# TritonDataCenter/containerpilot

Hardware: NVIDIA H100
Metric: events/sec through Bus.Publish (deliveries/s = 32-byte records landed in subscriber mailboxes) (higher is better)
Workload: dtype u8

## Files before the change

containerpilot_b200/csrc/cpbus.cu:

```cuda
#include "cpbus_kernels.cuh"

#include <algorithm>
#include <chrono>
#include <cstdio>
#include <cstdlib>
#include <cstring>
#include <deque>
#include <mutex>
#include <new>
#include <string>
#include <thread>
#include <unordered_map>
#include <vector>

using namespace cpbus_dev;

namespace {

thread_local char g_cuda_err[256] = "";

#define CK(call)                                                                                   \
  do {                                                                                             \
    cudaError_t e_ = (call);                                                                       \
    if (e_ != cudaSuccess) {                                                                       \
// ... 43 lines not shown
  uint32_t N = 0, R = 0, B = 0, K = 0;
  int store = CPBUS_STORE_V8;
  bool lossless = false, use_digest = false;

  cpbus_event* d_ring = nullptr;
  SubCtl* d_ctl = nullptr;
  DevTimer* d_timers = nullptr;
  DevStats* d_stats = nullptr;
  uint64_t* d_pow = nullptr;
  unsigned char* d_desc = nullptr;
  unsigned long long* d_desc_ready = nullptr;
  unsigned long long launch_seq = 0;
  cpbus_event* d_batch_local = nullptr;
  cpbus_event* d_admit_batch = nullptr;
  static constexpr int kPrefetch = 3;
  cpbus_event* d_prefetch[kPrefetch] = {};
  const void* pf_ptr[kPrefetch] = {};
  size_t pf_n[kPrefetch] = {};
  unsigned long long pf_seq[kPrefetch] = {};
  int pf_next = 0;
  std::vector<void*> shared_owned, shared_mapped;
  unsigned long long* d_pf_state = nullptr;
  cpbus_event* d_pf_buf = nullptr;
  unsigned int* h_err = nullptr;
  unsigned int* d_err = nullptr;
  uint32_t stream_spin_us = 0;
  DevPubAcct* d_acct = nullptr;
  DevPubAcct* h_acct = nullptr;
  std::deque<DbgItem> dbg_pending;
  PairCounter pub_pairs;
  cpbus_event* d_drain = nullptr; size_t drain_cap = 0;
  uint2* d_drain_idx = nullptr; size_t drain_idx_cap = 0;
  unsigned long long* d_ready_lb = nullptr; size_t ready_lb_tiles = 0;
  cpbus_ready* d_ready = nullptr; uint32_t* d_ready_slot = nullptr; size_t ready_stage_cap = 0;
  unsigned long long* h_ready_hdr = nullptr;
  unsigned long long* d_ready_hdr = nullptr;
  uint32_t subs_per_warp = 0;
  uint32_t order_block = 0;
  bool order_heavy_first = true;
  bool pdl = true;
  int h2d_spin_us = 30;
  bool zero_copy = false;
  cudaEvent_t launched = nullptr;
  int hints = -1;
  static constexpr int kFoldSlots = 8;
  unsigned long long* d_fold = nullptr;
  cudaEvent_t fold_done[kFoldSlots] = {};
  uint32_t fold_next = 0;
  static constexpr int kStage = 8;
  static constexpr int kEpoch = 4;
  static constexpr int kDevSlots = 64, kDevEpoch = 16;
  cpbus_event* d_stage = nullptr;
  cudaEvent_t epoch_done[kDevSlots / kDevEpoch] = {};
  uint32_t dev_slot = 0;
  cpbus_event* h_batch[kStage] = {};
  cudaEvent_t h2d_done[kStage] = {};
  cudaEvent_t consumed[kStage] = {};
  cudaStream_t copy_stream = nullptr;
  cudaStream_t result_stream = nullptr;
  DevResultSlot* d_result = nullptr;
  DevResultSlot* h_result = nullptr;
  cudaEvent_t result_done[8] = {};
  uint32_t result_next = 0;
  DevStats* h_stats = nullptr;
  unsigned long long* h_fold = nullptr;
  int cur = 0;
  size_t n_staged = 0;

  std::vector<uint32_t> h_mask;
  std::vector<uint8_t> h_active;
  std::vector<uint8_t> h_npairs;
  uint2* d_pairs = nullptr;
  uint32_t n_paired = 0;
  uint32_t* d_order = nullptr;
  uint32_t n_order = 0, n_filtered = 0;
  bool order_dirty = true;
  int use_order = 1;
  std::vector<size_t> oneshot_idx;
  std::vector<HostTimer> h_timers;
  uint32_t n_next = 0, n_active = 0, n_timers = 0;
  uint64_t min_period = UINT64_MAX;

  uint64_t now = 0, last_watermark = 0, seq = 0;
  uint64_t room_lb = 0;

  int dbg_head = -1, dbg_tail = 0;
  cpbus_event dbg[10]{};

  std::unordered_map<std::string, uint32_t> intern;
  std::vector<std::string> sources;
  size_t intern_bytes = 0;
  struct EphSlot { std::string s; uint32_t gen = 0; bool live = false; };
  std::vector<EphSlot> eph;
  std::unordered_map<std::string, uint32_t> eph_map;
  uint32_t eph_next = 0;
  uint64_t eph_live = 0, eph_recycled = 0;
  std::vector<cpbus_stream*> streams;

  cpbus_stats_t st{};
  std::mutex mu;
};

namespace {
// ... 459 lines not shown
  ALLOC(b->d_pf_buf, (size_t)kStreamPrefetch * B * sizeof(cpbus_event)); ALLOC(b->d_pf_state, 64);
  ALLOC(b->d_acct, sizeof(DevPubAcct));
  if (cudaMemsetAsync(b->d_pf_state, 0, 64, b->stream) != cudaSuccess ||
      cudaMemsetAsync(b->d_acct, 0, sizeof(DevPubAcct), b->stream) != cudaSuccess) return fail(CPBUS_ECUDA);
  if (cudaHostAlloc((void**)&b->h_err, 64, cudaHostAllocMapped) != cudaSuccess) return fail(CPBUS_ENOMEM);
  memset(b->h_err, 0, 64);
  if (cudaHostGetDevicePointer((void**)&b->d_err, b->h_err, 0) != cudaSuccess) return fail(CPBUS_ECUDA);
  if (cudaMallocHost((void**)&b->h_acct, offsetof(DevPubAcct, pair_key)) != cudaSuccess) return fail(CPBUS_ENOMEM);
  for (int i = 0; i < cpbus::kPrefetch; i++) ALLOC(b->d_prefetch[i], (size_t)B * sizeof(cpbus_event));
  ALLOC(b->d_result, sizeof(DevResultSlot) * kResultRing * kResultSub);
  if (cudaMemsetAsync(b->d_result, 0, sizeof(DevResultSlot) * kResultRing * kResultSub, b->stream) != cudaSuccess) return fail(CPBUS_ECUDA);
  if (cudaMallocHost((void**)&b->h_result, sizeof(DevResultSlot) * 8 * kResultSub) != cudaSuccess) return fail(CPBUS_ENOMEM);
  for (int i = 0; i < 8; i++)
    if (cudaEventCreateWithFlags(&b->result_done[i], cudaEventDisableTiming) != cudaSuccess) return fail(CPBUS_ECUDA);
#undef ALLOC
  if (cudaMallocHost((void**)&b->h_stats, sizeof(DevStats)) != cudaSuccess) return fail(CPBUS_ENOMEM);
  if (cudaMallocHost((void**)&b->h_fold, 32 * cpbus::kFoldSlots) != cudaSuccess) return fail(CPBUS_ENOMEM);
  for (int i = 0; i < cpbus::kFoldSlots; i++)
    if (cudaEventCreateWithFlags(&b->fold_done[i], cudaEventDisableTiming) != cudaSuccess) return fail(CPBUS_ECUDA);
  bool ok = cudaMemsetAsync(b->d_ctl, 0, N * sizeof(SubCtl), b->stream) == cudaSuccess &&
            cudaMemsetAsync(b->d_stats, 0, sizeof(DevStats), b->stream) == cudaSuccess &&
            (!K || cudaMemsetAsync(b->d_timers, 0xFF, N * K * sizeof(DevTimer), b->stream) == cudaSuccess) &&
            cudaStreamSynchronize(b->stream) == cudaSuccess;
  if (!ok) return fail(CPBUS_ECUDA);
  {
    std::vector<uint64_t> pw(kPowTableLen);
    uint64_t x = 1;
    for (uint32_t i = 0; i < kPowTableLen; i++) { pw[i] = x; x *= kDigestP; }
    if (cudaMemcpyAsync(b->d_pow, pw.data(), kPowTableLen * 8, cudaMemcpyHostToDevice, b->stream) != cudaSuccess ||
        cudaStreamSynchronize(b->stream) != cudaSuccess) return fail(CPBUS_ECUDA);
  }
  b->h_mask.assign(N, 0);
  b->h_active.assign(N, 0);
  b->intern.emplace(std::string(), 0u);
  b->sources.emplace_back();
  *out = b;
  return CPBUS_OK;
} CPBUS_CATCH

int cpbus_destroy(cpbus_t* b) try {
  if (!b) return CPBUS_EINVAL;
  cudaSetDevice(b->device);
  if (b->stream) cudaStreamSynchronize(b->stream);
  while (!b->streams.empty()) cpbus_stream_close(b->streams.back());
  cudaFree(b->d_ring); cudaFree(b->d_ctl); cudaFree(b->d_order); cudaFree(b->d_pairs);
  cudaFree(b->d_timers); cudaFree(b->d_stats); cudaFree(b->d_fold); cudaFree(b->d_pow); cudaFree(b->d_desc); cudaFree(b->d_desc_ready);
  if (b->copy_stream) cudaStreamSynchronize(b->copy_stream);
  if (b->result_stream) { cudaStreamSynchronize(b->result_stream); cudaStreamDestroy(b->result_stream); }
  for (int i = 0; i < cpbus::kStage; i++) {
    if (b->h_batch[i]) cudaFreeHost(b->h_batch[i]);
    if (b->h2d_done[i]) cudaEventDestroy(b->h2d_done[i]);
    if (b->consumed[i]) cudaEventDestroy(b->consumed[i]);
  }
  cudaFree(b->d_stage);
  for (int i = 0; i < cpbus::kDevSlots / cpbus::kDevEpoch; i++) if (b->epoch_done[i]) cudaEventDestroy(b->epoch_done[i]);
  if (b->copy_stream) cudaStreamDestroy(b->copy_stream);
  if (b->launched) cudaEventDestroy(b->launched);
  cudaFree(b->d_drain); cudaFree(b->d_drain_idx);
  cudaFree(b->d_ready_lb); cudaFree(b->d_ready); cudaFree(b->d_ready_slot);
  if (b->h_ready_hdr) cudaFreeHost(b->h_ready_hdr);
  cudaFree(b->d_result); cudaFree(b->d_batch_local); cudaFree(b->d_admit_batch); cudaFree(b->d_pf_buf); cudaFree(b->d_pf_state); cudaFree(b->d_acct);
  if (b->h_err) cudaFreeHost(b->h_err);
  if (b->h_acct) cudaFreeHost(b->h_acct);
  for (int i = 0; i < cpbus::kPrefetch; i++) cudaFree(b->d_prefetch[i]);
  for (void* p : b->shared_mapped) cudaIpcCloseMemHandle(p);
  for (void* p : b->shared_owned) cudaFree(p);
// ... 42 lines not shown
  b->eph_map.emplace(std::move(key), slot);
  *source_id = CPBUS_EPHEMERAL_BIT | ((e.gen & 0x7FFFu) << 16) | slot;
  return CPBUS_OK;
} CPBUS_CATCH

int cpbus_source(cpbus_t* b, uint32_t id, char* out, size_t cap, size_t* len) try {
  if (!b) return CPBUS_EINVAL;
  if (id & CPBUS_EPHEMERAL_BIT) {
    const uint32_t slot = id & 0xFFFFu, gen = (id >> 16) & 0x7FFFu;
    if (slot >= b->eph.size() || !b->eph[slot].live || (b->eph[slot].gen & 0x7FFFu) != gen) return CPBUS_ENOENT;
    const std::string& s = b->eph[slot].s;
    if (len) *len = s.size();
    if (out && cap) memcpy(out, s.data(), std::min(cap, s.size()));
    return CPBUS_OK;
  }
  if (id >= b->sources.size()) return CPBUS_ENOENT;
  const std::string& s = b->sources[id];
  if (len) *len = s.size();
  if (out && cap) memcpy(out, s.data(), std::min(cap, s.size()));
  return CPBUS_OK;
} CPBUS_CATCH

int cpbus_subscribe_many(cpbus_t* b, const uint32_t* masks, uint32_t n, uint32_t* first_sub_id) try {
  if (!b || !n) return CPBUS_EINVAL;
  if ((uint64_t)b->n_next + n > b->N) return CPBUS_ENOSPC;
  int rc = dev_guard(b); if (rc) return rc;
  if ((rc = flush_staged(b, b->now))) return rc;
  const uint32_t first = b->n_next;
  std::vector<SubCtl> blocks(n);
  memset(blocks.data(), 0, (size_t)n * sizeof(SubCtl));
  for (uint32_t i = 0; i < n; i++) {
    b->h_mask[first + i] = (masks ? masks[i] : CPBUS_MASK_ALL) & CPBUS_MASK_ALL;
    blocks[i].mask = b->h_mask[first + i] | kActiveBit;
    b->h_active[first + i] = 1;
    if (b->h_mask[first + i] != CPBUS_MASK_ALL) b->n_filtered++;
  }
  CK(cudaMemcpyAsync(b->d_ctl + first, blocks.data(), (size_t)n * sizeof(SubCtl), cudaMemcpyHostToDevice, b->stream));
  CK(cudaStreamSynchronize(b->stream));
  b->n_next += n; b->n_active += n; b->order_dirty = true;
  if (first_sub_id) *first_sub_id = b->cfg.sub_id_base + first;
  return CPBUS_OK;
} CPBUS_CATCH

int cpbus_subscribe(cpbus_t* b, uint32_t mask, uint32_t* sub_id) { return cpbus_subscribe_many(b, &mask, 1, sub_id); }

static int push_mask_words(cpbus* b, uint32_t first, uint32_t n);

int cpbus_subscribe_pairs(cpbus_t* b, uint32_t mask, const cpbus_pair* pairs, uint32_t n_pairs, uint32_t* sub_id) try {
  if (!b || n_pairs > CPBUS_MAX_PAIRS || (n_pairs && !pairs)) return CPBUS_EINVAL;
  for (uint32_t j = 0; j < n_pairs; j++) if (pairs[j].code >= CPBUS_N_CODES) return CPBUS_EINVAL;
  uint2 row[CPBUS_MAX_PAIRS];
  uint32_t used = 0;
  for (uint32_t j = 0; j < n_pairs; j++)
    if (!((mask >> pairs[j].code) & 1u)) row[used++] = make_uint2(pairs[j].code, pairs[j].source_id);
  if (used == 0) return cpbus_subscribe_many(b, &mask, 1, sub_id);
  int rc = dev_guard(b); if (rc) return rc;
  if (!b->d_pairs) {
    if (cudaMalloc((void**)&b->d_pairs, (size_t)b->N * CPBUS_MAX_PAIRS * sizeof(uint2)) != cudaSuccess) {
      snprintf(g_cuda_err, sizeof(g_cuda_err), "cudaMalloc(pair tables) failed");
      return CPBUS_ENOMEM;
    }
    CK(cudaMemsetAsync(b->d_pairs, 0xFF, (size_t)b->N * CPBUS_MAX_PAIRS * sizeof(uint2), b->stream));
    b->h_npairs.assign(b->N, 0);
  }
  uint32_t id = 0;
  if ((rc = cpbus_subscribe_many(b, &mask, 1, &id))) return rc;
  const uint32_t l = id - b->cfg.sub_id_base;
  for (uint32_t j = used; j < CPBUS_MAX_PAIRS; j++) row[j] = make_uint2(kPairNone, kPairNone);
  CK(cudaMemcpyAsync(b->d_pairs + (size_t)l * CPBUS_MAX_PAIRS, row, sizeof(row), cudaMemcpyHostToDevice, b->stream));
// ... 696 lines not shown
  if (*(volatile unsigned int*)b->h_err) return CPBUS_ETIMEDOUT;
  if (!st->h_agree) {
    StreamAgreeResult *h = nullptr, *d = nullptr;
    CK(cudaHostAlloc((void**)&h, sizeof(StreamAgreeResult), cudaHostAllocMapped));
    if (cudaHostGetDevicePointer((void**)&d, h, 0) != cudaSuccess) { cudaFreeHost(h); CK(cudaGetLastError()); return CPBUS_ECUDA; }
    st->h_agree = h; st->d_agree = d;
  }
  if (!st->agree_done) CK(cudaEventCreateWithFlags(&st->agree_done, cudaEventDisableTiming));
  const unsigned long long r = st->agree_round + 1;
  stream_agree_kernel<<<1, kStreamMaxConsumers, 0, b->stream>>>(st->ack, st->n_consumers, r, b->stream_spin_us, st->d_agree, b->d_err);
  CK(cudaGetLastError());
  b->st.kernel_launches++;
  st->agree_round = r; st->offered = false;
  CK(cudaEventRecord(st->agree_done, b->stream));
  CK(cudaEventSynchronize(st->agree_done));
  const volatile StreamAgreeResult* res = st->h_agree;
  if (res->status) return CPBUS_ETIMEDOUT;
  if (res->stalled) return CPBUS_EAGAIN;
  *m = res->m;
  return CPBUS_OK;
} CPBUS_CATCH

static int read_cursors(cpbus* b, uint32_t l, uint64_t* tail, uint64_t* head, uint64_t* lost = nullptr) {
  SubCtl c{};
  CK(cudaMemcpyAsync(&c, b->d_ctl + l, sizeof(SubCtl), cudaMemcpyDeviceToHost, b->stream));
  CK(cudaStreamSynchronize(b->stream));
  *tail = c.tail;
  *head = (!b->lossless && c.tail > b->R && c.tail - b->R > c.head) ? c.tail - b->R : c.head;
  if (lost) *lost = *head - c.head;
  return CPBUS_OK;
}

static int copy_slots(cpbus* b, uint32_t l, uint64_t from, size_t n, cpbus_event* out) {
  const cpbus_event* ring = b->d_ring + (size_t)l * b->R;
  const uint32_t s0 = (uint32_t)(from & (b->R - 1));
  const size_t first = std::min<size_t>(n, b->R - s0);
  if (first) CK(cudaMemcpyAsync(out, ring + s0, first * sizeof(cpbus_event), cudaMemcpyDeviceToHost, b->stream));
  if (n > first) CK(cudaMemcpyAsync(out + first, ring, (n - first) * sizeof(cpbus_event), cudaMemcpyDeviceToHost, b->stream));
  CK(cudaStreamSynchronize(b->stream));
  return CPBUS_OK;
}

int cpbus_drain(cpbus_t* b, uint32_t sub_id, cpbus_event* out, size_t cap, size_t* n, uint64_t* lost) try {
  if (!b || !n || (!out && cap)) return CPBUS_EINVAL;
  const uint32_t l = sub_id - b->cfg.sub_id_base;
  if (sub_id < b->cfg.sub_id_base || l >= b->n_next) return CPBUS_ENOENT;
  std::lock_guard<std::mutex> g(b->mu);
  int rc = dev_guard(b); if (rc) return rc;
  uint64_t tail = 0, head = 0;
  uint64_t gone = 0;
  if ((rc = read_cursors(b, l, &tail, &head, &gone))) return rc;
  if (lost) *lost = gone;
  const size_t take = (size_t)std::min<uint64_t>(tail - head, cap);
  if (take && (rc = copy_slots(b, l, head, take, out))) return rc;
  head += take;
  CK(cudaMemcpyAsync(&b->d_ctl[l].head, &head, 8, cudaMemcpyHostToDevice, b->stream));
  CK(cudaStreamSynchronize(b->stream));
  *n = take;
  return CPBUS_OK;
} CPBUS_CATCH

int cpbus_drain_many(cpbus_t* b, uint32_t first_sub, uint32_t n, cpbus_event* out, size_t cap, uint32_t* offsets,
                     uint32_t* counts, size_t* total) try {
  if (!b || !n || !out || !cap || !offsets || !counts || !total || cap > 0xFFFFFFFFull) return CPBUS_EINVAL;
  const uint32_t l = first_sub - b->cfg.sub_id_base;
  if (first_sub < b->cfg.sub_id_base || (uint64_t)l + n > b->n_next) return CPBUS_ENOENT;
  std::lock_guard<std::mutex> g(b->mu);
// ... 11 lines not shown
  b->st.kernel_launches++;
  std::vector<uint2> idx(n);
  CK(cudaMemcpyAsync(idx.data(), b->d_drain_idx, (size_t)n * sizeof(uint2), cudaMemcpyDeviceToHost, b->stream));
  CK(cudaStreamSynchronize(b->stream));
  size_t tot = 0, hi = 0;
  for (uint32_t i = 0; i < n; i++) {
    offsets[i] = idx[i].x; counts[i] = idx[i].y; tot += idx[i].y;
    hi = std::max<size_t>(hi, (size_t)idx[i].x + idx[i].y);
  }
  if (hi) CK(cudaMemcpyAsync(out, b->d_drain, hi * sizeof(cpbus_event), cudaMemcpyDeviceToHost, b->stream));
  CK(cudaStreamSynchronize(b->stream));
  *total = tot;
  return CPBUS_OK;
} CPBUS_CATCH

int cpbus_drain_ready(cpbus_t* b, uint32_t first_sub, uint32_t n, uint32_t start_sub, cpbus_event* out, size_t cap,
                      cpbus_ready* ready, size_t ready_cap, size_t* n_ready, size_t* total, uint32_t* next_sub) try {
  if (!b || !out || !ready || !n_ready || !total || !next_sub || !n || !ready_cap) return CPBUS_EINVAL;
  if (cap < b->R || cap > 0xFFFFFFFFull) return CPBUS_EINVAL;
  if (start_sub < first_sub || start_sub - first_sub >= n) return CPBUS_EINVAL;
  const uint32_t l = first_sub - b->cfg.sub_id_base;
  if (first_sub < b->cfg.sub_id_base || (uint64_t)l + n > b->n_next) return CPBUS_ENOENT;
  std::lock_guard<std::mutex> g(b->mu);
  int rc = dev_guard(b); if (rc) return rc;
  const size_t rcap = std::min<size_t>(ready_cap, n);
  const uint32_t tiles = (n + kReadyTile - 1) / kReadyTile;
  if (b->drain_cap < cap) {
    cudaFree(b->d_drain); b->d_drain = nullptr; b->drain_cap = 0;
    CK(cudaMalloc((void**)&b->d_drain, cap * sizeof(cpbus_event))); b->drain_cap = cap;
  }
  if (b->ready_stage_cap < rcap) {
    cudaFree(b->d_ready); cudaFree(b->d_ready_slot); b->d_ready = nullptr; b->d_ready_slot = nullptr; b->ready_stage_cap = 0;
    CK(cudaMalloc((void**)&b->d_ready, rcap * sizeof(cpbus_ready)));
    CK(cudaMalloc((void**)&b->d_ready_slot, rcap * sizeof(uint32_t)));
    b->ready_stage_cap = rcap;
  }
  if (b->ready_lb_tiles < tiles) {
    cudaFree(b->d_ready_lb); b->d_ready_lb = nullptr; b->ready_lb_tiles = 0;
    CK(cudaMalloc((void**)&b->d_ready_lb, (kReadyLbOffset + (size_t)tiles) * sizeof(unsigned long long)));
    b->ready_lb_tiles = tiles;
  }
  if (!b->h_ready_hdr) {
    unsigned long long *h = nullptr, *d = nullptr;
    CK(cudaHostAlloc((void**)&h, 64, cudaHostAllocMapped));
    if (cudaHostGetDevicePointer((void**)&d, h, 0) != cudaSuccess) { cudaFreeHost(h); CK(cudaGetLastError()); return CPBUS_ECUDA; }
    b->h_ready_hdr = h; b->d_ready_hdr = d;
  }
  CK(cudaMemsetAsync(b->d_ready_lb + kReadyHdrWords, 0, (kReadyLbOffset - kReadyHdrWords + (size_t)tiles) * sizeof(unsigned long long),
                     b->stream));
  const uint32_t rot = start_sub - first_sub;
  drain_ready_scan_kernel<<<tiles, kThreads, 0, b->stream>>>(b->d_ctl, l, n, rot, b->R, b->lossless ? 1u : 0u, b->cfg.sub_id_base,
                                                              cap, rcap, b->d_ready_lb, b->d_ready, b->d_ready_slot);
  CK(cudaGetLastError());
  const uint32_t gather_grid = (uint32_t)std::min<size_t>((size_t)b->sm_count * 4, (rcap + kWarpsPerCta - 1) / kWarpsPerCta);
  drain_ready_gather_kernel<<<gather_grid, kThreads, 0, b->stream>>>(b->d_ring, b->R, b->cfg.sub_id_base, b->d_ready,
                                                                      b->d_ready_slot, b->d_ready_lb, b->d_drain, b->d_ready_hdr);
  CK(cudaGetLastError());
  b->st.kernel_launches += 2;
  CK(cudaStreamSynchronize(b->stream));
  const size_t nr = (size_t)b->h_ready_hdr[0], tot = (size_t)b->h_ready_hdr[1];
  const uint64_t cut = b->h_ready_hdr[2];
  if (nr) {
    CK(cudaMemcpyAsync(ready, b->d_ready, nr * sizeof(cpbus_ready), cudaMemcpyDeviceToHost, b->stream));
    CK(cudaMemcpyAsync(out, b->d_drain, tot * sizeof(cpbus_event), cudaMemcpyDeviceToHost, b->stream));
    CK(cudaStreamSynchronize(b->stream));
  }
  *n_ready = nr; *total = tot;
  *next_sub = cut >= n ? start_sub : first_sub + (uint32_t)((rot + cut) % n);
  return CPBUS_OK;
} CPBUS_CATCH

int cpbus_consume_all(cpbus_t* b) try {
  if (!b) return CPBUS_EINVAL;
  std::lock_guard<std::mutex> g(b->mu);
  int rc = dev_guard(b); if (rc) return rc;
  if (b->n_next) {
    const uint32_t threads = 256, grid = std::min<uint32_t>((b->n_next + threads - 1) / threads, (uint32_t)b->sm_count * 8);
    consume_all_kernel<<<grid, threads, 0, b->stream>>>(b->d_ctl, b->n_next);
    CK(cudaGetLastError());
    b->st.kernel_launches++;
  }
  b->room_lb = b->R;
  return CPBUS_OK;
} CPBUS_CATCH

int cpbus_peek_window(cpbus_t* b, uint32_t sub_id, cpbus_event* out, size_t cap, size_t* n) try {
  if (!b || !n || (!out && cap)) return CPBUS_EINVAL;
  const uint32_t l = sub_id - b->cfg.sub_id_base;
// ... 173 lines not shown
```

containerpilot_b200/csrc/cpbus_kernels.cuh:

```cuda
#pragma once
#include <cstdint>
#include <cuda_runtime.h>

#include "../../include/cpbus.h"

namespace cpbus_dev {

constexpr int kWarpsPerCta = 8;
constexpr int kThreads = kWarpsPerCta * 32;
#ifndef CPBUS_CTAS_PER_SM
#define CPBUS_CTAS_PER_SM 4
#endif
#ifndef CPBUS_SWIZZLE
#define CPBUS_SWIZZLE 2
#endif
#ifndef CPBUS_TICKS_REG
#define CPBUS_TICKS_REG 1
#endif
#ifndef CPBUS_COLD_EARLY
#define CPBUS_COLD_EARLY 1
#endif
#ifndef CPBUS_UNROLL2
#define CPBUS_UNROLL2 1
#endif
// ... 29 lines not shown
};
constexpr uint64_t kTimerIdle = ~0ull;

constexpr int kStatSlots = 256;
struct __align__(32) DevStatSlot { unsigned long long deliveries, ticks, pad[2]; };
struct DevStats {
  DevStatSlot slot[kStatSlots];
  unsigned long long admit_overflow, overwritten;
  unsigned long long admit_max_used;
  unsigned long long admit_deficit;
};

constexpr uint32_t kAcctPairSlots = 1u << 19;
constexpr int kAcctDbgRing = 64, kAcctDbgKeep = 10;
struct __align__(32) DevDbgTail {
  unsigned long long launch_seq;
  uint32_t n_broadcast, n_kept;
  cpbus_event ev[kAcctDbgKeep];
  uint32_t pad[4];
};
struct DevPubAcct {
  unsigned long long by_code[32];
  unsigned long long pair_overflow, pad[3];
  DevDbgTail tail[kAcctDbgRing];
  unsigned long long pair_key[kAcctPairSlots];
  unsigned long long pair_cnt[kAcctPairSlots];
};

struct __align__(32) SubCtl {
  unsigned long long tail;
  unsigned long long head;
  unsigned long long digest;
  uint32_t mask;
  uint32_t pad;
};

constexpr int kResultRing = 64, kResultSub = 8;
struct __align__(32) DevResultSlot { unsigned long long deliveries, ticks, digest_sum, launch_seq; };

struct __align__(32) StreamHdr { unsigned long long seq, watermark; uint32_t n, pad[3]; };
struct __align__(32) StreamMeta { uint32_t magic, n_slots, batch_cap, n_consumers, pad[4]; };
constexpr uint32_t kStreamMagic = 0x53425043u;
constexpr uint32_t kStreamMaxConsumers = 64;
constexpr int kStreamPrefetch = 3;
constexpr unsigned int kErrStreamTimeout = 1u, kErrStreamShape = 2u;
__host__ __device__ inline size_t stream_hdr_off() { return sizeof(StreamMeta); }
__host__ __device__ inline size_t stream_ack_off(uint32_t n_slots) { return stream_hdr_off() + (size_t)n_slots * sizeof(StreamHdr); }
__host__ __device__ inline size_t stream_payload_off(uint32_t n_slots) { return stream_ack_off(n_slots) + (size_t)kStreamMaxConsumers * 32; }
__host__ __device__ inline size_t stream_bytes(uint32_t n_slots, uint32_t batch_cap) { return stream_payload_off(n_slots) + (size_t)n_slots * batch_cap * 32; }

constexpr unsigned long long kOfferRoundMask = (1ull << 31) - 1;
__host__ __device__ inline uint32_t stream_offer_word_index(uint32_t consumer, unsigned long long round) {
  return 4u * consumer + 1u + (uint32_t)(round & 1ull);
}
__host__ __device__ inline unsigned long long stream_offer_word(unsigned long long round, uint32_t stalled, uint32_t prefix) {
  return ((round & kOfferRoundMask) << 33) | ((unsigned long long)(stalled ? 1u : 0u) << 32) | prefix;
}
struct __align__(16) StreamAgreeResult { uint32_t m, stalled, status, pad; };

struct FanoutParams {
  const cpbus_event* batch;
  cpbus_event* ring;
  SubCtl* ctl;
  DevTimer* timers;
  DevStats* stats;
  const uint64_t* pow_table;
  unsigned char* desc;
// ... 439 lines not shown
            uint32_t cbit[4];
#pragma unroll
            for (uint32_t u = 0; u < 4; u++) {
              const uint32_t i = (c0 + u) * 32 + lane;
              cbit[u] = i < n ? s_meta[i].x : 0u;
            }
#pragma unroll
            for (uint32_t u = 0; u < 4; u++) {
              const bool match = (m & cbit[u]) != 0;
              const uint32_t w = __ballot_sync(0xffffffffu, match);
              if (match) my_idx[base + __popc(w & ((1u << lane) - 1u))] = (uint16_t)((c0 + u) * 32 + lane);
              base += __popc(w);
            }
          }
          k = base;
          __syncwarp();
        }
        uint64_t acc = 0;
        for (uint32_t o0 = 0; o0 < k; o0 += 64) {
          const uint32_t o = o0 + lane;
          const bool v0 = o < k, v1 = o + 32 < k;
          uint32_t i0 = o, i1 = o + 32;
          if (!dense) { i0 = v0 ? my_idx[o] : 0u; i1 = v1 ? my_idx[o + 32] : 0u; }
          uint4 a0, b0, a1, b1;
          if (v0) lds_record<true, PLANAR>(s4r, i0, swr, a0, b0, hi_off);
          if (v1) lds_record<true, PLANAR>(s4r, i1, swr, a1, b1, hi_off);
          if (DIGEST && !dense) {
            if (v0) acc = acc * p32 + s_rhash[i0];
            if (v1) acc = acc * p32 + s_rhash[i1];
          }
#pragma unroll 2
          for (uint32_t t = j; t < j + L; t++) {
            const uint32_t tl = __shfl_sync(0xffffffffu, ma.x, t);
            const uint32_t id = __shfl_sync(0xffffffffu, my_ids, t);
            cpbus_event* ring = p.ring + (size_t)id * p.ring_cap;
            if (v0) st_v8(ring + ((tl + o) & Rm_r), a0, b0);
            if (v1) st_v8(ring + ((tl + o + 32) & Rm_r), a1, b1);
          }
        }
        uint64_t dsum = 0;
        if (DIGEST && k) {
          if (dense) dsum = s_q[n];
          else {
            const uint32_t cnt = k > (uint32_t)lane ? (k - lane + 31u) / 32u : 0u;
            dsum = cnt ? acc * s_pow[k - 1 - (lane + 32u * (cnt - 1u))] : 0ull;
            dsum = warp_sum64(dsum);
          }
        }
        if (k && (uint32_t)lane >= j && (uint32_t)lane < j + L) {
          const uint64_t tail = ((uint64_t)ma.y << 32) | ma.x, dig = ((uint64_t)mb.y << 32) | mb.x;
          const uint64_t nt = tail + k;
          const uint64_t nd = DIGEST ? dig * s_pow[k] + dsum : dig;
          st_sector(p.ctl + my_ids, make_uint4((uint32_t)nt, (uint32_t)(nt >> 32), ma.z, ma.w),
                    make_uint4((uint32_t)nd, (uint32_t)(nd >> 32), mb.z, 0u), keep);
          atomicAdd(&s_sum->acc_deliv, k);
          if (DIGEST) {
            const uint32_t f = (uint32_t)nd ^ (uint32_t)(nd >> 32);
            atomicAdd(&s_sum->acc_dig_lo, f & 0xFFFFu);
            atomicAdd(&s_sum->acc_dig_hi, f >> 16);
          }
        }
        __syncwarp();
        j += L;
      }
    }
  }
  if (runs_done) pos = pos_end;
  uint4 ca = make_uint4(0, 0, 0, 0), cb = ca, ta = ca;
  if (ORDERED && pos < pos_end) ld_sector(p.ctl + s, ca, cb, keep);
  const uint32_t present = s_dsum[0];
  const bool has_unicast = s_dsum[1] != 0;
  bool bulk_pending = false;
  uint32_t tri_blk = blockIdx.x * kWarpsPerCta + warp, tri_base = 0, tri_live = 0;
  uint4 tri_a = make_uint4(0, 0, 0, 0), tri_b = tri_a;
  uint32_t rnd_first = rng_first, rnd_phase = 0;
  for (;;) {
  if constexpr (STAGED) {
    if (aborted || rnd_first >= rng_end) break;
    stage_round(rnd_first);
    mbar_wait(&s_sum->mbar_state, rnd_phase);
    rnd_phase ^= 1u;
    pos = rnd_first + warp; pos_end = rnd_first + min(p.stage_subs, rng_end - rnd_first);
  }
  if constexpr (PAIRS) {
    bool exhausted = aborted;
    while (!tri_live && !exhausted) {
      tri_base = tri_blk * 32u;
// ... 35 lines not shown
    tri_live &= tri_live - 1u;
    pos = tri_base + jl; pos_end = pos + 1u; s = pos;
    ca = make_uint4(__shfl_sync(0xffffffffu, tri_a.x, jl), __shfl_sync(0xffffffffu, tri_a.y, jl), __shfl_sync(0xffffffffu, tri_a.z, jl), __shfl_sync(0xffffffffu, tri_a.w, jl));
    cb = make_uint4(__shfl_sync(0xffffffffu, tri_b.x, jl), __shfl_sync(0xffffffffu, tri_b.y, jl), __shfl_sync(0xffffffffu, tri_b.z, jl), __shfl_sync(0xffffffffu, tri_b.w, jl));
    if (timers_on && tk_slot < K) ld_half(p.timers + (size_t)s * K + tk_slot, ta, keep);
  }
  const uint32_t Rm = p.ring_cap - 1;
  const uint4* s4 = reinterpret_cast<const uint4*>(s_batch);
  const uint32_t scratch_words = max(32u, cap / 2u);
  uint32_t* my_tick = s_tick + warp * scratch_words;

  uint32_t run_mask = 0xffffffffu, run_k = 0;
  uint64_t run_sum = 0;
  for (; pos < pos_end; pos += pos_step) {
    const uint32_t si = pos - rnd_first;
    uint4 cur_a = ca, cur_b = cb;
    auto ctl_half = [&](uint32_t h) -> uint4 { return STAGED ? s_ctl4[2u * si + h] : (h ? cur_b : cur_a); };
    auto tim_half = [&](uint32_t h) -> uint4 {
      if (STAGED) return s_tim4[2u * (si * K + tk_slot) + h];
      if (!h) return ta;
      uint4 cold;
      ld_half(reinterpret_cast<const unsigned char*>(p.timers + (size_t)s * K + tk_slot) + 16, cold, keep);
      return cold;
    };
    if (STAGED) { cur_a = ctl_half(0); cur_b = ctl_half(1); }
    if (ORDERED) s = __shfl_sync(0xffffffffu, my_ids, (pos - pos0) & 31); else s = pos;
    if (ORDERED) {
      const uint32_t pn = pos + pos_step;
      if (pn < pos_end) ld_sector(p.ctl + __shfl_sync(0xffffffffu, my_ids, (pn - pos0) & 31), ca, cb, keep);
    }
    const uint32_t m = cur_b.z;
    if (!(m & kActiveBit)) continue;
    const uint64_t tail = ((uint64_t)cur_a.y << 32) | cur_a.x;
    cpbus_event* ring = p.ring + (size_t)s * p.ring_cap;
    const uint32_t gid = p.sub_base + s;
    const uint32_t nslots = timers_on ? min((m >> kTimerHintShift) & 0xFu, K) : 0u;
    const bool dense = !has_unicast && ((m & present) == present);

    uint32_t n_ticks = 0, tk_mask = 0, tk_rank = 0, tk_src = 0, tk_fired = 0;
    bool tk_valid = false; uint64_t tk_due = 0, tk_period = 0;
    if (nslots) {
      uint64_t tk_due0 = kTimerIdle;
      if (TIMERS && tk_slot < nslots) {
        const uint4 hot = tim_half(0);
        tk_due0 = ((uint64_t)hot.y << 32) | hot.x; tk_period = ((uint64_t)hot.w << 32) | hot.z;
      }
      tk_due = tk_due0 + (uint64_t)tk_j * tk_period;
      tk_valid = tk_due0 != kTimerIdle && tk_due <= p.w_now && (tk_j == 0 || tk_period != 0);
      tk_mask = __ballot_sync(0xffffffffu, tk_valid);
      n_ticks = __popc(tk_mask);
      if (n_ticks) {

        if (J == 32 || (tk_mask >> J) == 0) tk_rank = tk_j;
        else {
#pragma unroll 1
          for (int t = 0; t < 32; t++) {
            if (!((tk_mask >> t) & 1u)) continue;
            const uint64_t od = shfl64(tk_due, t);
            const uint32_t os = __shfl_sync(0xffffffffu, tk_slot, t);
            tk_rank += (od < tk_due || (od == tk_due && os < tk_slot)) ? 1u : 0u;
          }
        }
      }
    }
    uint32_t tk_pos = 0;
    if (tk_valid) {
      uint32_t lo = 0, hi = n;
// ... 250 lines not shown
          tk_src = cold.x; tk_fired = cold.y;
        }
      }
      if (tk_valid) {
        const uint32_t out = tk_mp + tk_rank;
        const uint64_t w0 = (uint64_t)tk_fired + tk_j, w1 = tk_due;
        const uint64_t w2 = (uint64_t)CPBUS_TIMER_EXPIRED | ((uint64_t)tk_src << 32);
        const uint64_t w3 = (uint64_t)gid | ((uint64_t)CPBUS_F_TICK << 32);
        const uint4 a = make_uint4((uint32_t)w0, (uint32_t)(w0 >> 32), (uint32_t)w1, (uint32_t)(w1 >> 32));
        const uint4 b = make_uint4((uint32_t)w2, (uint32_t)(w2 >> 32), (uint32_t)w3, (uint32_t)(w3 >> 32));
        st_v8(ring + (((uint32_t)tail + out) & Rm), a, b);
        if (DIGEST) dsum += record_hash_words(w0, w1, w2, w3) * s_pow[k - 1 - out];
      }
      if (DIGEST) dsum = warp_sum64(dsum);
      __syncwarp();
    }

    if (n_ticks) {
      const uint32_t slotmask = (J == 32 ? 0xffffffffu : ((1u << J) - 1u)) << (tk_slot * J);
      const uint32_t fired_here = __popc(tk_mask & slotmask);
      if (TIMERS && tk_j == 0 && tk_slot < nslots && fired_here) {
        unsigned char* t = reinterpret_cast<unsigned char*>(&p.timers[(size_t)s * K + tk_slot]);
        const uint64_t nd = tk_period ? tk_due + (uint64_t)fired_here * tk_period : kTimerIdle;
        st_half(t, make_uint4((uint32_t)nd, (uint32_t)(nd >> 32), (uint32_t)tk_period, (uint32_t)(tk_period >> 32)), keep);
        st_half(t + 16, make_uint4(tk_src, tk_fired + fired_here, 0u, 0u), keep);
      }
    }
    if (lane == 0 && k) {
      const uint4 c0 = ctl_half(0), c1 = ctl_half(1);
      const uint64_t dig = ((uint64_t)c1.y << 32) | c1.x;
      const uint64_t nt = tail + k;
      const uint64_t nd = DIGEST ? dig * s_pow[k] + dsum : dig;
      st_sector(p.ctl + s, make_uint4((uint32_t)nt, (uint32_t)(nt >> 32), c0.z, c0.w),
                make_uint4((uint32_t)nd, (uint32_t)(nd >> 32), m, 0u), keep);
      atomicAdd(&s_sum->acc_deliv, k);
      if (DIGEST) {
        const uint32_t f = (uint32_t)nd ^ (uint32_t)(nd >> 32);
        atomicAdd(&s_sum->acc_dig_lo, f & 0xFFFFu);
        atomicAdd(&s_sum->acc_dig_hi, f >> 16);
      }
      if (TIMERS && n_ticks) atomicAdd(&s_sum->acc_ticks, n_ticks);
    }
  }

  if constexpr (ORDERED) break;
  if constexpr (STAGED) {
    __syncthreads();
    rnd_first += p.stage_subs;
  }
  }
  if (STORE == CPBUS_STORE_BULK && bulk_pending && lane == 0)
    asm volatile("cp.async.bulk.wait_group 0;" ::: "memory");
  __syncthreads();
  if (tid == 0) {
    DevStatSlot* st = &p.stats->slot[blockIdx.x % kStatSlots];
    if (s_sum->acc_deliv) atomicAdd(&st->deliveries, (unsigned long long)s_sum->acc_deliv);
    if (s_sum->acc_ticks) atomicAdd(&st->ticks, (unsigned long long)s_sum->acc_ticks);
    DevResultSlot* rs = &p.result[blockIdx.x % kResultSub];
    if (s_sum->acc_deliv) atomicAdd(&rs->deliveries, (unsigned long long)s_sum->acc_deliv);
    if (s_sum->acc_ticks) atomicAdd(&rs->ticks, (unsigned long long)s_sum->acc_ticks);
    if (s_sum->acc_dig_lo | s_sum->acc_dig_hi) atomicAdd(&rs->digest_sum, (unsigned long long)s_sum->acc_dig_lo + ((unsigned long long)s_sum->acc_dig_hi << 16));
    if (blockIdx.x == 0) atomicAdd(&rs->launch_seq, p.launch_seq);
  }
  if (blockIdx.x == 0 && p.acct && !aborted) {
    if (tid < 32 && tid != CPBUS_METRIC && s_dsum[2 + tid]) atomicAdd(&p.acct->by_code[tid], (unsigned long long)s_dsum[2 + tid]);
    for (uint32_t i = tid; i < n; i += kThreads) {
      if (s_meta[i].y != CPBUS_TARGET_ALL) continue;
// ... 145 lines not shown
  __syncthreads();
  if (threadIdx.x == 0 && s_max) atomicMax(&stats->admit_max_used, s_max);
}

__global__ void consume_all_kernel(SubCtl* ctl, uint32_t n) {
  for (uint32_t i = blockIdx.x * blockDim.x + threadIdx.x; i < n; i += gridDim.x * blockDim.x) ctl[i].head = ctl[i].tail;
}

__global__ void overwritten_kernel(const SubCtl* ctl, uint32_t n, uint32_t ring_cap, unsigned long long* out) {
  unsigned long long acc = 0;
  for (uint32_t i = blockIdx.x * blockDim.x + threadIdx.x; i < n; i += gridDim.x * blockDim.x) {
    const SubCtl c = ctl[i];
    if (c.tail > ring_cap && c.tail - ring_cap > c.head) acc += c.tail - ring_cap - c.head;
  }
  acc = warp_sum64(acc);
  if ((threadIdx.x & 31) == 0 && acc) atomicAdd(out, acc);
}

__global__ void drain_many_kernel(SubCtl* ctl, const cpbus_event* ring, uint32_t first, uint32_t n, uint32_t ring_cap,
                                  uint32_t lossless, cpbus_event* out, uint32_t out_cap, uint2* index, unsigned int* cursor) {
  const uint32_t lane = threadIdx.x & 31;
  const uint32_t w = (blockIdx.x * blockDim.x + threadIdx.x) >> 5, nw = (gridDim.x * blockDim.x) >> 5;
  for (uint32_t i = w; i < n; i += nw) {
    SubCtl* c = ctl + first + i;
    const unsigned long long tail = c->tail;
    unsigned long long head = c->head;
    if (!lossless && tail > ring_cap && tail - ring_cap > head) head = tail - ring_cap;
    const uint32_t avail = (uint32_t)(tail - head);
    uint32_t off = 0;
    if (lane == 0 && avail) off = atomicAdd(cursor, avail);
    off = __shfl_sync(0xffffffffu, off, 0);
    const bool fits = avail && off + avail <= out_cap;
    if (fits) {
      const cpbus_event* r = ring + (size_t)(first + i) * ring_cap;
      for (uint32_t j = lane; j < avail; j += 32) {
        const uint4* src = reinterpret_cast<const uint4*>(r + ((head + j) & (ring_cap - 1)));
        uint4* dst = reinterpret_cast<uint4*>(out + off + j);
        dst[0] = src[0]; dst[1] = src[1];
      }
    }
    if (lane == 0) {
      index[i] = make_uint2(fits ? off : 0u, fits ? avail : 0u);
      if (fits) c->head = tail;
    }
  }
}

constexpr uint32_t kReadyItems = 4, kReadyTile = kThreads * kReadyItems;
static_assert(kReadyItems * kWarpsPerCta == 32, "one lane per (item, warp) chunk of a tile");
constexpr unsigned long long kLbAgg = 1ull << 62, kLbIncl = 2ull << 62, kLbRecMax = (1ull << 33) - 1;
constexpr uint32_t kReadyHdrWords = 4, kReadyLbOffset = 8;

__device__ __forceinline__ unsigned long long lb_pack(unsigned long long flag, unsigned long long ready, unsigned long long rec) {
  return flag | (ready << 33) | (rec < kLbRecMax ? rec : kLbRecMax);
}

__global__ void __launch_bounds__(kThreads) drain_ready_scan_kernel(SubCtl* __restrict__ ctl, uint32_t first, uint32_t n,
                                                                    uint32_t rot, uint32_t ring_cap, uint32_t lossless,
                                                                    uint32_t sub_base, unsigned long long cap,
                                                                    unsigned long long ready_cap, unsigned long long* lb,
                                                                    cpbus_ready* __restrict__ ready, uint32_t* __restrict__ slot) {
  __shared__ uint32_t s_tile;
  __shared__ uint32_t s_wr[32];
  __shared__ unsigned long long s_wc[32];
  __shared__ unsigned long long s_base_r, s_base_c;
  unsigned long long* hdr = lb;
  unsigned long long* status = lb + kReadyLbOffset;
  const uint32_t lane = threadIdx.x & 31, warp = threadIdx.x >> 5;
  if (threadIdx.x == 0) s_tile = atomicAdd(reinterpret_cast<unsigned int*>(lb + kReadyHdrWords), 1u);
  __syncthreads();
  const uint32_t tile = s_tile;
  uint32_t loc[kReadyItems], r_in[kReadyItems];
  unsigned long long tl[kReadyItems], cur[kReadyItems], hd[kReadyItems], c_in[kReadyItems];
#pragma unroll
  for (uint32_t k = 0; k < kReadyItems; k++) {
    const uint32_t p = tile * kReadyTile + k * kThreads + threadIdx.x;
    unsigned long long t = 0, h = 0, c = 0;
    uint32_t l = 0;
    if (p < n) {
      unsigned long long q = (unsigned long long)rot + p;
      if (q >= n) q -= n;
      l = first + (uint32_t)q;
      const ulonglong2 th = *reinterpret_cast<const ulonglong2*>(ctl + l);
      t = th.x; h = th.y; c = h;
      if (!lossless && t > ring_cap && t - ring_cap > c) c = t - ring_cap;
    }
    loc[k] = l; tl[k] = t; hd[k] = h; cur[k] = c;
    uint32_t r = t != c ? 1u : 0u;
    unsigned long long s = t - c;
#pragma unroll
    for (int o = 1; o < 32; o <<= 1) {
      const uint32_t ro = __shfl_up_sync(0xffffffffu, r, o);
      const unsigned long long so = shfl64(s, (int)lane - o);
      if ((int)lane >= o) { r += ro; s += so; }
// ... 21 lines not shown
    } else {
      if (lane == 0) *reinterpret_cast<volatile unsigned long long*>(status + tile) = lb_pack(kLbAgg, agg_r, agg_c);
      for (int pred = (int)tile - 1;; pred -= 32) {
        const int j = pred - (int)lane;
        unsigned long long v = kLbIncl;
        do {
          if (j >= 0) v = *reinterpret_cast<volatile unsigned long long*>(status + j);
        } while (__any_sync(0xffffffffu, (v >> 62) == 0));
        const uint32_t incl = __ballot_sync(0xffffffffu, (v >> 62) == 2);
        const uint32_t stop = incl ? (uint32_t)(__ffs(incl) - 1) : 31u;
        ex_r += warp_sum64(lane <= stop ? (v >> 33) & ((1ull << 29) - 1) : 0ull);
        ex_c += warp_sum64(lane <= stop ? v & kLbRecMax : 0ull);
        ex_c = ex_c < kLbRecMax ? ex_c : kLbRecMax;
        if (incl) break;
      }
      if (lane == 0) *reinterpret_cast<volatile unsigned long long*>(status + tile) = lb_pack(kLbIncl, ex_r + agg_r, ex_c + agg_c);
    }
    if (lane == 0) {
      s_base_r = ex_r; s_base_c = ex_c;
      const unsigned long long all_r = ex_r + agg_r, all_c = ex_c + agg_c;
      if (tile == gridDim.x - 1 && all_r <= ready_cap && all_c <= cap) { hdr[0] = all_r; hdr[1] = all_c; hdr[2] = n; }
    }
  }
  __syncthreads();
#pragma unroll
  for (uint32_t k = 0; k < kReadyItems; k++) {
    const unsigned long long cnt = tl[k] - cur[k];
    if (!cnt) continue;
    const uint32_t chunk = k * kWarpsPerCta + warp;
    const unsigned long long r = s_base_r + s_wr[chunk] + r_in[k] - 1;
    const unsigned long long o = s_base_c + s_wc[chunk] + c_in[k] - cnt;
    if (r < ready_cap && o + cnt <= cap) {
      ready[r] = cpbus_ready{sub_base + loc[k], (uint32_t)cnt, (uint32_t)o, 0u, cur[k] - hd[k]};
      slot[r] = (uint32_t)(cur[k] & (ring_cap - 1));
      ctl[loc[k]].head = tl[k];
    } else if (r == 0 || (r - 1 < ready_cap && o <= cap)) {
      hdr[0] = r; hdr[1] = o; hdr[2] = tile * kReadyTile + k * kThreads + threadIdx.x;
    }
  }
}

__global__ void __launch_bounds__(kThreads) drain_ready_gather_kernel(const cpbus_event* __restrict__ ring, uint32_t ring_cap,
                                                                      uint32_t sub_base, const cpbus_ready* __restrict__ ready,
                                                                      const uint32_t* __restrict__ slot,
                                                                      const unsigned long long* __restrict__ hdr,
                                                                      cpbus_event* __restrict__ out, unsigned long long* h_hdr) {
  const unsigned long long n_ready = hdr[0];
  if (blockIdx.x == 0 && threadIdx.x < 3) h_hdr[threadIdx.x] = hdr[threadIdx.x];
  const uint32_t lane = threadIdx.x & 31, half = lane & 1;
  const unsigned long long nw = (gridDim.x * blockDim.x) >> 5;
  for (unsigned long long e = (blockIdx.x * blockDim.x + threadIdx.x) >> 5; e < n_ready; e += nw) {
    const cpbus_ready rd = ready[e];
    const uint32_t s0 = slot[e];
    const uint4* src = reinterpret_cast<const uint4*>(ring + (size_t)(rd.sub_id - sub_base) * ring_cap);
    uint4* dst = reinterpret_cast<uint4*>(out + rd.offset);
    uint32_t j = lane >> 1;
    for (; j + 16 < rd.count; j += 32) {
      const uint4 a = src[2 * ((s0 + j) & (ring_cap - 1)) + half], b = src[2 * ((s0 + j + 16) & (ring_cap - 1)) + half];
      dst[2 * j + half] = a; dst[2 * (j + 16) + half] = b;
    }
    if (j < rd.count) dst[2 * j + half] = src[2 * ((s0 + j) & (ring_cap - 1)) + half];
  }
}

__global__ void digest_fold_kernel(const SubCtl* ctl, uint32_t first, uint32_t n, uint32_t sub_base,
                                   unsigned long long* out4) {
  unsigned long long c = 0, d = 0, x = 0;
  for (uint32_t i = blockIdx.x * blockDim.x + threadIdx.x; i < n; i += gridDim.x * blockDim.x) {
    const unsigned long long t = ctl[first + i].tail, g = ctl[first + i].digest;
    c += t; d += g;
    x ^= record_hash_words(g, t, sub_base + first + i, 0);
  }
  c = warp_sum64(c); d = warp_sum64(d);
#pragma unroll
  for (int o = 16; o > 0; o >>= 1) {
    uint32_t lo = __shfl_xor_sync(0xffffffffu, (uint32_t)x, o), hi = __shfl_xor_sync(0xffffffffu, (uint32_t)(x >> 32), o);
    x ^= ((unsigned long long)hi << 32) | lo;
  }
  if ((threadIdx.x & 31) == 0) { atomicAdd(&out4[0], c); atomicAdd(&out4[1], d); atomicXor(&out4[2], x); }
  if (blockIdx.x == 0 && threadIdx.x == 0) out4[3] = n;
}

__global__ void stream_offer_kernel(unsigned long long* word, unsigned long long value) {
  asm volatile("st.release.sys.global.u64 [%0], %1;" ::"l"(word), "l"(value) : "memory");
}

__global__ void __launch_bounds__(kStreamMaxConsumers) stream_agree_kernel(const unsigned long long* ack, uint32_t n_consumers,
// ... 38 lines not shown
```

Baseline: 92.60 billion.

## Decouple subscriber ring placement from subscriber id via mask-ordered ring slots

Adds a per-subscriber ring_slot field, stored in the former pad word of SubCtl, so each subscriber's ring buffer location is chosen at subscribe time. Rings are ordered by the same mask ordering used for publish, so subscribers processed together write to adjacent rings. The publish, drain and gather kernels and the host copy path all index rings through ring_slot instead of the subscriber index. This aims to improve write locality during fan-out, at the cost of an extra indirection and a wider slot array in the drain path.

```diff
diff --git a/containerpilot_b200/csrc/cpbus.cu b/containerpilot_b200/csrc/cpbus.cu
--- a/containerpilot_b200/csrc/cpbus.cu
+++ b/containerpilot_b200/csrc/cpbus.cu
@@ -99,7 +99,7 @@
   cpbus_event* d_drain = nullptr; size_t drain_cap = 0;
   uint2* d_drain_idx = nullptr; size_t drain_idx_cap = 0;
   unsigned long long* d_ready_lb = nullptr; size_t ready_lb_tiles = 0;
-  cpbus_ready* d_ready = nullptr; uint32_t* d_ready_slot = nullptr; size_t ready_stage_cap = 0;
+  cpbus_ready* d_ready = nullptr; uint2* d_ready_slot = nullptr; size_t ready_stage_cap = 0;
   unsigned long long* h_ready_hdr = nullptr;
   unsigned long long* d_ready_hdr = nullptr;
   uint32_t subs_per_warp = 0;
@@ -136,6 +136,7 @@
 
   std::vector<uint32_t> h_mask;
   std::vector<uint8_t> h_active;
+  std::vector<uint32_t> h_ring_slot;
   std::vector<uint8_t> h_npairs;
   uint2* d_pairs = nullptr;
   uint32_t n_paired = 0;
@@ -661,6 +662,7 @@
   }
   b->h_mask.assign(N, 0);
   b->h_active.assign(N, 0);
+  b->h_ring_slot.assign(N, 0);
   b->intern.emplace(std::string(), 0u);
   b->sources.emplace_back();
   *out = b;
@@ -769,9 +771,16 @@
   for (uint32_t i = 0; i < n; i++) {
     b->h_mask[first + i] = (masks ? masks[i] : CPBUS_MASK_ALL) & CPBUS_MASK_ALL;
     blocks[i].mask = b->h_mask[first + i] | kActiveBit;
+    blocks[i].ring_slot = first + i;
     b->h_active[first + i] = 1;
     if (b->h_mask[first + i] != CPBUS_MASK_ALL) b->n_filtered++;
   }
+  if (b->K == 0 && n > 1) {
+    std::vector<uint32_t> order;
+    mask_order(b->h_mask.data() + first, nullptr, n, b->R, b->order_block, b->order_heavy_first, order);
+    for (uint32_t k = 0; k < n; k++) blocks[order[k]].ring_slot = first + k;
+  }
+  for (uint32_t i = 0; i < n; i++) b->h_ring_slot[first + i] = blocks[i].ring_slot;
   CK(cudaMemcpyAsync(b->d_ctl + first, blocks.data(), (size_t)n * sizeof(SubCtl), cudaMemcpyHostToDevice, b->stream));
   CK(cudaStreamSynchronize(b->stream));
   b->n_next += n; b->n_active += n; b->order_dirty = true;
@@ -1534,7 +1543,7 @@
 }
 
 static int copy_slots(cpbus* b, uint32_t l, uint64_t from, size_t n, cpbus_event* out) {
-  const cpbus_event* ring = b->d_ring + (size_t)l * b->R;
+  const cpbus_event* ring = b->d_ring + (size_t)b->h_ring_slot[l] * b->R;
   const uint32_t s0 = (uint32_t)(from & (b->R - 1));
   const size_t first = std::min<size_t>(n, b->R - s0);
   if (first) CK(cudaMemcpyAsync(out, ring + s0, first * sizeof(cpbus_event), cudaMemcpyDeviceToHost, b->stream));
@@ -1612,7 +1621,7 @@
   if (b->ready_stage_cap < rcap) {
     cudaFree(b->d_ready); cudaFree(b->d_ready_slot); b->d_ready = nullptr; b->d_ready_slot = nullptr; b->ready_stage_cap = 0;
     CK(cudaMalloc((void**)&b->d_ready, rcap * sizeof(cpbus_ready)));
-    CK(cudaMalloc((void**)&b->d_ready_slot, rcap * sizeof(uint32_t)));
+    CK(cudaMalloc((void**)&b->d_ready_slot, rcap * sizeof(uint2)));
     b->ready_stage_cap = rcap;
   }
   if (b->ready_lb_tiles < tiles) {
@@ -1633,7 +1642,7 @@
                                                               cap, rcap, b->d_ready_lb, b->d_ready, b->d_ready_slot);
   CK(cudaGetLastError());
   const uint32_t gather_grid = (uint32_t)std::min<size_t>((size_t)b->sm_count * 4, (rcap + kWarpsPerCta - 1) / kWarpsPerCta);
-  drain_ready_gather_kernel<<<gather_grid, kThreads, 0, b->stream>>>(b->d_ring, b->R, b->cfg.sub_id_base, b->d_ready,
+  drain_ready_gather_kernel<<<gather_grid, kThreads, 0, b->stream>>>(b->d_ring, b->R, b->d_ready,
                                                                       b->d_ready_slot, b->d_ready_lb, b->d_drain, b->d_ready_hdr);
   CK(cudaGetLastError());
   b->st.kernel_launches += 2;
diff --git a/containerpilot_b200/csrc/cpbus_kernels.cuh b/containerpilot_b200/csrc/cpbus_kernels.cuh
--- a/containerpilot_b200/csrc/cpbus_kernels.cuh
+++ b/containerpilot_b200/csrc/cpbus_kernels.cuh
@@ -85,7 +85,7 @@
   unsigned long long head;
   unsigned long long digest;
   uint32_t mask;
-  uint32_t pad;
+  uint32_t ring_slot;
 };
 
 constexpr int kResultRing = 64, kResultSub = 8;
@@ -591,8 +591,8 @@
 #pragma unroll 2
           for (uint32_t t = j; t < j + L; t++) {
             const uint32_t tl = __shfl_sync(0xffffffffu, ma.x, t);
-            const uint32_t id = __shfl_sync(0xffffffffu, my_ids, t);
-            cpbus_event* ring = p.ring + (size_t)id * p.ring_cap;
+            const uint32_t rs = __shfl_sync(0xffffffffu, mb.w, t);
+            cpbus_event* ring = p.ring + (size_t)rs * p.ring_cap;
             if (v0) st_v8(ring + ((tl + o) & Rm_r), a0, b0);
             if (v1) st_v8(ring + ((tl + o + 32) & Rm_r), a1, b1);
           }
@@ -611,7 +611,7 @@
           const uint64_t nt = tail + k;
           const uint64_t nd = DIGEST ? dig * s_pow[k] + dsum : dig;
           st_sector(p.ctl + my_ids, make_uint4((uint32_t)nt, (uint32_t)(nt >> 32), ma.z, ma.w),
-                    make_uint4((uint32_t)nd, (uint32_t)(nd >> 32), mb.z, 0u), keep);
+                    make_uint4((uint32_t)nd, (uint32_t)(nd >> 32), mb.z, mb.w), keep);
           atomicAdd(&s_sum->acc_deliv, k);
           if (DIGEST) {
             const uint32_t f = (uint32_t)nd ^ (uint32_t)(nd >> 32);
@@ -713,7 +713,7 @@
     const uint32_t m = cur_b.z;
     if (!(m & kActiveBit)) continue;
     const uint64_t tail = ((uint64_t)cur_a.y << 32) | cur_a.x;
-    cpbus_event* ring = p.ring + (size_t)s * p.ring_cap;
+    cpbus_event* ring = p.ring + (size_t)(PAIRS ? p.ctl[s].ring_slot : cur_b.w) * p.ring_cap;
     const uint32_t gid = p.sub_base + s;
     const uint32_t nslots = timers_on ? min((m >> kTimerHintShift) & 0xFu, K) : 0u;
     const bool dense = !has_unicast && ((m & present) == present);
@@ -1030,7 +1030,7 @@
       const uint64_t nt = tail + k;
       const uint64_t nd = DIGEST ? dig * s_pow[k] + dsum : dig;
       st_sector(p.ctl + s, make_uint4((uint32_t)nt, (uint32_t)(nt >> 32), c0.z, c0.w),
-                make_uint4((uint32_t)nd, (uint32_t)(nd >> 32), m, 0u), keep);
+                make_uint4((uint32_t)nd, (uint32_t)(nd >> 32), m, PAIRS ? p.ctl[s].ring_slot : c1.w), keep);
       atomicAdd(&s_sum->acc_deliv, k);
       if (DIGEST) {
         const uint32_t f = (uint32_t)nd ^ (uint32_t)(nd >> 32);
@@ -1242,7 +1242,7 @@
     off = __shfl_sync(0xffffffffu, off, 0);
     const bool fits = avail && off + avail <= out_cap;
     if (fits) {
-      const cpbus_event* r = ring + (size_t)(first + i) * ring_cap;
+      const cpbus_event* r = ring + (size_t)c->ring_slot * ring_cap;
       for (uint32_t j = lane; j < avail; j += 32) {
         const uint4* src = reinterpret_cast<const uint4*>(r + ((head + j) & (ring_cap - 1)));
         uint4* dst = reinterpret_cast<uint4*>(out + off + j);
@@ -1269,7 +1269,7 @@
                                                                     uint32_t rot, uint32_t ring_cap, uint32_t lossless,
                                                                     uint32_t sub_base, unsigned long long cap,
                                                                     unsigned long long ready_cap, unsigned long long* lb,
-                                                                    cpbus_ready* __restrict__ ready, uint32_t* __restrict__ slot) {
+                                                                    cpbus_ready* __restrict__ ready, uint2* __restrict__ slot) {
   __shared__ uint32_t s_tile;
   __shared__ uint32_t s_wr[32];
   __shared__ unsigned long long s_wc[32];
@@ -1357,7 +1357,7 @@
     const unsigned long long o = s_base_c + s_wc[chunk] + c_in[k] - cnt;
     if (r < ready_cap && o + cnt <= cap) {
       ready[r] = cpbus_ready{sub_base + loc[k], (uint32_t)cnt, (uint32_t)o, 0u, cur[k] - hd[k]};
-      slot[r] = (uint32_t)(cur[k] & (ring_cap - 1));
+      slot[r] = make_uint2(ctl[loc[k]].ring_slot, (uint32_t)(cur[k] & (ring_cap - 1)));
       ctl[loc[k]].head = tl[k];
     } else if (r == 0 || (r - 1 < ready_cap && o <= cap)) {
       hdr[0] = r; hdr[1] = o; hdr[2] = tile * kReadyTile + k * kThreads + threadIdx.x;
@@ -1366,8 +1366,8 @@
 }
 
 __global__ void __launch_bounds__(kThreads) drain_ready_gather_kernel(const cpbus_event* __restrict__ ring, uint32_t ring_cap,
-                                                                      uint32_t sub_base, const cpbus_ready* __restrict__ ready,
-                                                                      const uint32_t* __restrict__ slot,
+                                                                      const cpbus_ready* __restrict__ ready,
+                                                                      const uint2* __restrict__ slot,
                                                                       const unsigned long long* __restrict__ hdr,
                                                                       cpbus_event* __restrict__ out, unsigned long long* h_hdr) {
   const unsigned long long n_ready = hdr[0];
@@ -1376,8 +1376,9 @@
   const unsigned long long nw = (gridDim.x * blockDim.x) >> 5;
   for (unsigned long long e = (blockIdx.x * blockDim.x + threadIdx.x) >> 5; e < n_ready; e += nw) {
     const cpbus_ready rd = ready[e];
-    const uint32_t s0 = slot[e];
-    const uint4* src = reinterpret_cast<const uint4*>(ring + (size_t)(rd.sub_id - sub_base) * ring_cap);
+    const uint2 sl = slot[e];
+    const uint32_t s0 = sl.y;
+    const uint4* src = reinterpret_cast<const uint4*>(ring + (size_t)sl.x * ring_cap);
     uint4* dst = reinterpret_cast<uint4*>(out + rd.offset);
     uint32_t j = lane >> 1;
     for (; j + 16 < rd.count; j += 32) {
```

New measurement: 92.58 billion, median of 6. About the same (-0.0%).
